# AliyunContainerService/gpushare-device-plugin

Measured on AMD Instinct MI355X. Metric: pods/sec scheduled (gpu-mem share Allocate pipeline), higher is better.
Workload: dtype n/a; 1 GPU; model=gpushare-device-plugin (MI355X), global_batch=4, seq_len=71, parallelism=1 plugin + 1 churn ranks, pods_allocated=2776, pods_failed=0

## Files before the change

__graft_entry__.py:

```python

from __future__ import annotations

import os
import sys

sys.path.insert(0, os.path.dirname(os.path.abspath(__file__)))


def build() -> None:
    os.environ.setdefault("PYTORCH_ROCM_ARCH", "gfx950")
    from gpushare_amd.native.build import build as native_build

    native_build()
    import gpushare_amd
    import gpushare_amd._amdsmi
    import gpushare_amd._devlist
    import gpushare_amd._httprt

    import gpushare_amd._canary

    print("[graft] build OK: _amdsmi, _devlist, _httprt, _canary importable")


def smoke() -> None:
    import tempfile

    import torch

    assert torch.cuda.is_available(), "torch sees no GPU"

    import gpushare_amd._canary as canary
    from gpushare_amd import consts
    from gpushare_amd.allocator import Allocator
    from gpushare_amd.cluster.kubeclient import FakeKubeClient
    from gpushare_amd.cluster.podmanager import PodManager
    from gpushare_amd.device.amdsmi_source import AmdSmiSource
    from gpushare_amd.deviceplugin.server import GPUSharePlugin
    from gpushare_amd.deviceplugin.stubkubelet import StubKubelet

    src = AmdSmiSource()
    gpus = src.devices()
    assert gpus, "no AMD GPUs enumerated"
    g0 = gpus[0]
    print(
        f"[graft] {len(gpus)} GPU(s); GPU0 uuid={g0.uuid} "
        f"vram={g0.memory_bytes >> 30} GiB render={g0.render_path}"
    )

    result = canary.probe(0, vram_probe_mb=64, bandwidth=False)
    print(f"[graft] canary: {result}")
    assert result["ok"], f"canary probe failed: {result}"

    with tempfile.TemporaryDirectory(prefix="gpushare-smoke-") as sockdir:
        kube = FakeKubeClient(node_name="smoke-node")
# ... 37 lines not shown
```

gpushare_amd/deviceplugin/server.py:

```python

from __future__ import annotations

import logging
import os
import threading
import time
from concurrent import futures
from typing import Optional

import grpc

from .. import consts, metrics
from ..device import PhysicalGPU
from ..device.fakedev import FakeDeviceTable, make_codec
from . import v1beta1 as api

log = logging.getLogger(__name__)


class GPUSharePlugin:
    def __init__(
        self,
        gpus: list[PhysicalGPU],
        allocator,
        unit: str = consts.GIB,
        resource_name: str = consts.RESOURCE_NAME,
        socket_dir: str = consts.DEVICE_PLUGIN_PATH,
        socket_name: str = consts.SERVER_SOCK_NAME,
        max_workers: int = 64,
        allow_oversize_inventory: bool = False,
        numa_topology: bool = False,
    ):
        self.gpus = gpus
        self.allocator = allocator
        self.unit = unit
        self.resource_name = resource_name
        self.socket_dir = socket_dir
        self.socket_name = socket_name
        self.socket_path = os.path.join(socket_dir, socket_name)
        self.max_workers = max_workers

        self.table = FakeDeviceTable.build(gpus, unit)
        self._codec = make_codec(
            self.table.ids,
            numa=self.table.numa_of if numa_topology else None,
        )
        metrics.observe_inventory(len(self.table))
        self.inventory_bytes = len(self._codec.encode([]))
        if self.inventory_bytes > consts.KUBELET_GRPC_MAX_MSG:
            msg = (
                f"inventory of {len(self.table)} fake devices encodes to "
                f"{self.inventory_bytes / 1e6:.1f} MB — over the kubelet's "
                f"4 MiB gRPC receive limit; use GiB granularity on "
                f"288 GiB-class GPUs (or a kubelet built with a larger "
                f"limit + allow_oversize_inventory)"
            )
            if not allow_oversize_inventory:
                raise ValueError(msg)
            log.warning("%s — continuing as requested", msg)

        self._health_lock = threading.Condition()
        self._unhealthy_gpus: set[int] = set()
        self._health_version = 0

        self._server: Optional[grpc.Server] = None
        self._stop_event = threading.Event()

    def set_gpu_health(self, gpu_index: Optional[int], healthy: bool) -> None:
        with self._health_lock:
            targets = (
                [g.index for g in self.gpus] if gpu_index is None else [gpu_index]
            )
            changed = False
            for idx in targets:
                if healthy and idx in self._unhealthy_gpus:
                    self._unhealthy_gpus.discard(idx)
                    changed = True
                elif not healthy and idx not in self._unhealthy_gpus:
                    self._unhealthy_gpus.add(idx)
                    changed = True
            if changed:
                self._health_version += 1
                self._health_lock.notify_all()
                metrics.observe_health_event(
                    "recovered" if healthy else "unhealthy",
                    len(self._unhealthy_gpus),
                )

    def _unhealthy_fake_indices(self) -> list[int]:
        out: list[int] = []
        for gpu_idx in self._unhealthy_gpus:
            out.extend(self.table.gpu_fake_indices(gpu_idx))
        return out

    def encoded_device_list(self) -> bytes:
        return self._codec.encode(self._unhealthy_fake_indices())

    def _get_options(self, request, context) -> "api.DevicePluginOptions":
# ... 44 lines not shown
                out.deviceIDs.extend(chosen[: cr.allocation_size])
                continue
            chosen_set = set(chosen)
            by_gpu: dict[int, list[str]] = {}
            for dev_id in cr.available_deviceIDs:
                if dev_id in chosen_set:
                    continue
                gpu_idx = self.table.gpu_of.get(dev_id)
                if gpu_idx is not None:
                    by_gpu.setdefault(gpu_idx, []).append(dev_id)
            fitting = sorted(
                (ids for ids in by_gpu.values() if len(ids) >= need),
                key=len,
            )
            if need and fitting:
                chosen.extend(fitting[0][:need])
            else:
                for ids in sorted(by_gpu.values(), key=len, reverse=True):
                    if need <= 0:
                        break
                    take = ids[:need]
                    chosen.extend(take)
                    need -= len(take)
            out.deviceIDs.extend(chosen)
        return resp

    def _pre_start(self, request, context) -> "api.PreStartContainerResponse":
        return api.PreStartContainerResponse()

    def start(self) -> None:
        if os.path.exists(self.socket_path):
            os.unlink(self.socket_path)
        os.makedirs(self.socket_dir, exist_ok=True)

        handlers = {
            "GetDevicePluginOptions": grpc.unary_unary_rpc_method_handler(
                self._get_options,
                request_deserializer=api.Empty.FromString,
                response_serializer=lambda m: m.SerializeToString(),
            ),
            "ListAndWatch": grpc.unary_stream_rpc_method_handler(
                self._list_and_watch,
                request_deserializer=api.Empty.FromString,
                response_serializer=None,
            ),
            "Allocate": grpc.unary_unary_rpc_method_handler(
                self._allocate,
                request_deserializer=api.AllocateRequest.FromString,
                response_serializer=lambda m: m.SerializeToString(),
            ),
            "PreStartContainer": grpc.unary_unary_rpc_method_handler(
                self._pre_start,
                request_deserializer=api.PreStartContainerRequest.FromString,
                response_serializer=lambda m: m.SerializeToString(),
            ),
            "GetPreferredAllocation": grpc.unary_unary_rpc_method_handler(
                self._get_preferred_allocation,
                request_deserializer=(
                    api.PreferredAllocationRequest.FromString
                ),
                response_serializer=lambda m: m.SerializeToString(),
            ),
        }
        self._server = grpc.server(
            futures.ThreadPoolExecutor(max_workers=self.max_workers)
        )
        self._server.add_generic_rpc_handlers(
            (
                grpc.method_handlers_generic_handler(
                    api.DEVICEPLUGIN_SERVICE, handlers
                ),
            )
        )
        self._server.add_insecure_port(f"unix://{self.socket_path}")
        self._stop_event.clear()
        self._server.start()

        with grpc.insecure_channel(f"unix://{self.socket_path}") as ch:
            grpc.channel_ready_future(ch).result(timeout=5)
        log.info("device plugin serving on %s", self.socket_path)

    def register(self, kubelet_socket: Optional[str] = None) -> None:
        if kubelet_socket is None:
            kubelet_socket = os.path.join(
                self.socket_dir, consts.KUBELET_SOCKET_NAME
            )
        req = api.RegisterRequest(
            version=consts.API_VERSION,
            endpoint=self.socket_name,
            resource_name=self.resource_name,
        )
        with grpc.insecure_channel(f"unix://{kubelet_socket}") as ch:
            grpc.channel_ready_future(ch).result(timeout=10)
            register = ch.unary_unary(
                api.METHOD_REGISTER,
                request_serializer=lambda m: m.SerializeToString(),
                response_deserializer=api.Empty.FromString,
            )
            register(req, timeout=10)
        log.info(
            "registered resource %s (%d fake devices) with kubelet at %s",
            self.resource_name,
            len(self.table),
            kubelet_socket,
        )

    def serve(self, kubelet_socket: Optional[str] = None) -> None:
        self.start()
        self.register(kubelet_socket)

    def stop(self) -> None:
        self._stop_event.set()
        with self._health_lock:
            self._health_lock.notify_all()
        if self._server is not None:
            self._server.stop(grace=1).wait(timeout=5)
            self._server = None
        if os.path.exists(self.socket_path):
            try:
                os.unlink(self.socket_path)
            except OSError:
                pass
        if hasattr(self.allocator, "close"):
            self.allocator.close()

    def wait_stopped(self, timeout: float = 5.0) -> None:
        deadline = time.monotonic() + timeout
        while self._server is not None and time.monotonic() < deadline:
            time.sleep(0.01)
```

gpushare_amd/native/build.py:

```python

from __future__ import annotations

import os
import subprocess
import sys
import sysconfig
from pathlib import Path

import pybind11

HERE = Path(__file__).resolve().parent
PKG = HERE.parent
EXT_SUFFIX = sysconfig.get_config_var("EXT_SUFFIX") or ".so"
ROCM = os.environ.get("ROCM_PATH", "/opt/rocm")
GPU_ARCH = os.environ.get("PYTORCH_ROCM_ARCH", "gfx950").split(";")[0]

_COMMON = [
    "-O2",
    "-std=c++17",
    "-fPIC",
    "-shared",
    "-fvisibility=hidden",
    f"-I{pybind11.get_include()}",
    f"-I{sysconfig.get_paths()['include']}",
]


def _needs_build(srcs: list[Path], out: Path, force: bool) -> bool:
    if force or not out.exists():
        return True
    return any(s.stat().st_mtime > out.stat().st_mtime for s in srcs)


def _run(cmd: list[str]) -> None:
    print("[native/build]", " ".join(cmd), flush=True)
    subprocess.run(cmd, check=True)


def build(force: bool = False, verbose: bool = True) -> list[Path]:
    built = []

    targets = [
        (
            "g++",
            HERE / "amdsmi_shim.cpp",
            PKG / f"_amdsmi{EXT_SUFFIX}",
            [f"-I{ROCM}/include", "-ldl"],
        ),
        ("g++", HERE / "devlist_codec.cpp", PKG / f"_devlist{EXT_SUFFIX}", []),
        ("g++", HERE / "http_rt.cpp", PKG / f"_httprt{EXT_SUFFIX}", []),
        (
            os.path.join(ROCM, "bin", "hipcc"),
            HERE / "canary.hip",
            PKG / f"_canary{EXT_SUFFIX}",
            [f"--offload-arch={GPU_ARCH}", "-O3"],
        ),
        (
            "g++",
            HERE / "memguard.cpp",
            PKG / "libgpushare_memguard.so",
            ["-fvisibility=default", "-ldl"],
        ),
    ]
    deps = {"http_rt.cpp": [HERE / "http_parse.h"]}
    for compiler, src, out, extra in targets:
        if not _needs_build([src, *deps.get(src.name, [])], out, force):
            continue
        _run([compiler, *_COMMON, str(src), "-o", str(out), *extra])
        built.append(out)
    return built


def main() -> None:
    force = "--force" in sys.argv
    built = build(force=force)
    print(f"[native/build] built {len(built)} extension(s)")
    sys.path.insert(0, str(PKG.parent))
    import gpushare_amd._amdsmi as smi
    import gpushare_amd._devlist as dl
    import gpushare_amd._httprt as rt

    print("[native/build] _amdsmi available:", smi.available())
    c = dl.DeviceListCodec(["amd-0-_-0"])
    assert len(c.encode()) > 0
    print("[native/build] _devlist OK")
    head = rt.build_head("GET", "/", "localhost", {"Accept": "*/*"})
    assert head.startswith(b"GET / HTTP/1.1\r\nHost: localhost\r\n")
    print("[native/build] _httprt OK")


if __name__ == "__main__":
    main()
```

Baseline: 2446 pods/s.

## Serve device-plugin gRPC through a native C++ HTTP/2 core instead of grpcio

Adds a pybind11 C++ extension that implements a minimal HTTP/2 + HPACK gRPC server over the Unix socket, with per-connection threads that call into Python handlers only for dispatch. The plugin uses it by default and falls back to grpcio if the module is missing or the env switch disables it. The aim is to cut grpcio's per-RPC Python and threadpool overhead on the Allocate path. In exchange it carries a hand-written protocol implementation with risks around correctness, flow control, thread lifetime and GIL handling.

```diff
diff --git a/__graft_entry__.py b/__graft_entry__.py
--- a/__graft_entry__.py
+++ b/__graft_entry__.py
@@ -15,11 +15,12 @@
     import gpushare_amd
     import gpushare_amd._amdsmi
     import gpushare_amd._devlist
+    import gpushare_amd._grpcsrv
     import gpushare_amd._httprt
 
     import gpushare_amd._canary
 
-    print("[graft] build OK: _amdsmi, _devlist, _httprt, _canary importable")
+    print("[graft] build OK: _amdsmi, _devlist, _httprt, _grpcsrv, _canary importable")
 
 
 def smoke() -> None:
diff --git a/gpushare_amd/deviceplugin/server.py b/gpushare_amd/deviceplugin/server.py
--- a/gpushare_amd/deviceplugin/server.py
+++ b/gpushare_amd/deviceplugin/server.py
@@ -16,6 +16,39 @@
 from . import v1beta1 as api
 
 log = logging.getLogger(__name__)
+
+
+def _native_core():
+    if os.environ.get("GPUSHARE_GRPC_NATIVE", "1") == "0":
+        return None
+    try:
+        from .. import _grpcsrv
+    except ImportError:
+        return None
+    return _grpcsrv
+
+
+class RpcAbort(Exception):
+
+    def __init__(self, code: int, details: str):
+        super().__init__(details)
+        self.grpc_code = code
+        self.grpc_details = details
+
+
+class _NativeContext:
+
+    __slots__ = ("_call",)
+
+    def __init__(self, call):
+        self._call = call
+
+    def is_active(self) -> bool:
+        return self._call.is_active()
+
+    def abort(self, code, details: str):
+        value = getattr(code, "value", code)
+        raise RpcAbort(value[0] if isinstance(value, tuple) else int(value), details)
 
 
 class GPUSharePlugin:
@@ -64,6 +97,7 @@
         self._health_version = 0
 
         self._server: Optional[grpc.Server] = None
+        self._native = None
         self._stop_event = threading.Event()
 
     def set_gpu_health(self, gpu_index: Optional[int], healthy: bool) -> None:
@@ -174,7 +208,62 @@
         if os.path.exists(self.socket_path):
             os.unlink(self.socket_path)
         os.makedirs(self.socket_dir, exist_ok=True)
-
+        self._stop_event.clear()
+        core = _native_core()
+        if core is not None:
+            self._start_native(core)
+        else:
+            self._start_grpcio()
+
+        with grpc.insecure_channel(f"unix://{self.socket_path}") as ch:
+            grpc.channel_ready_future(ch).result(timeout=5)
+        log.info(
+            "device plugin serving on %s (%s transport)",
+            self.socket_path,
+            "native" if self._native is not None else "grpcio",
+        )
+
+    def _start_native(self, core) -> None:
+        self._native_methods = {
+            api.METHOD_GET_OPTIONS: (
+                self._get_options, api.Empty.FromString, False),
+            api.METHOD_LIST_AND_WATCH: (
+                self._list_and_watch, api.Empty.FromString, True),
+            api.METHOD_ALLOCATE: (
+                self._allocate, api.AllocateRequest.FromString, False),
+            api.METHOD_PRE_START: (
+                self._pre_start,
+                api.PreStartContainerRequest.FromString, False),
+            api.METHOD_GET_PREFERRED: (
+                self._get_preferred_allocation,
+                api.PreferredAllocationRequest.FromString, False),
+        }
+        self._native = core.Server(
+            self.socket_path, self._native_dispatch,
+            consts.KUBELET_GRPC_MAX_MSG,
+        )
+        self._native.start()
+
+    def _native_dispatch(self, path: str, data: bytes, call):
+        method = self._native_methods.get(path)
+        if method is None:
+            raise RpcAbort(12, "Method not found!")
+        behavior, parse, streaming = method
+        try:
+            request = parse(data)
+        except Exception:
+            log.exception("Exception deserializing request!")
+            raise RpcAbort(13, "Exception deserializing request!") from None
+        try:
+            response = behavior(request, _NativeContext(call))
+        except RpcAbort:
+            raise
+        except Exception:
+            log.exception("Exception calling application")
+            raise
+        return response if streaming else response.SerializeToString()
+
+    def _start_grpcio(self) -> None:
         handlers = {
             "GetDevicePluginOptions": grpc.unary_unary_rpc_method_handler(
                 self._get_options,
@@ -215,12 +304,7 @@
             )
         )
         self._server.add_insecure_port(f"unix://{self.socket_path}")
-        self._stop_event.clear()
         self._server.start()
-
-        with grpc.insecure_channel(f"unix://{self.socket_path}") as ch:
-            grpc.channel_ready_future(ch).result(timeout=5)
-        log.info("device plugin serving on %s", self.socket_path)
 
     def register(self, kubelet_socket: Optional[str] = None) -> None:
         if kubelet_socket is None:
@@ -258,6 +342,10 @@
         if self._server is not None:
             self._server.stop(grace=1).wait(timeout=5)
             self._server = None
+        if self._native is not None:
+            if not self._native.stop(1.0):
+                log.warning("native gRPC core: threads still winding down")
+            self._native = None
         if os.path.exists(self.socket_path):
             try:
                 os.unlink(self.socket_path)
@@ -268,5 +356,7 @@
 
     def wait_stopped(self, timeout: float = 5.0) -> None:
         deadline = time.monotonic() + timeout
-        while self._server is not None and time.monotonic() < deadline:
+        while (
+            self._server is not None or self._native is not None
+        ) and time.monotonic() < deadline:
             time.sleep(0.01)
diff --git a/gpushare_amd/native/build.py b/gpushare_amd/native/build.py
--- a/gpushare_amd/native/build.py
+++ b/gpushare_amd/native/build.py
@@ -50,6 +50,12 @@
         ("g++", HERE / "devlist_codec.cpp", PKG / f"_devlist{EXT_SUFFIX}", []),
         ("g++", HERE / "http_rt.cpp", PKG / f"_httprt{EXT_SUFFIX}", []),
         (
+            "g++",
+            HERE / "grpc_srv.cpp",
+            PKG / f"_grpcsrv{EXT_SUFFIX}",
+            ["-pthread"],
+        ),
+        (
             os.path.join(ROCM, "bin", "hipcc"),
             HERE / "canary.hip",
             PKG / f"_canary{EXT_SUFFIX}",
@@ -62,7 +68,10 @@
             ["-fvisibility=default", "-ldl"],
         ),
     ]
-    deps = {"http_rt.cpp": [HERE / "http_parse.h"]}
+    deps = {
+        "http_rt.cpp": [HERE / "http_parse.h"],
+        "grpc_srv.cpp": [HERE / "h2_core.h"],
+    }
     for compiler, src, out, extra in targets:
         if not _needs_build([src, *deps.get(src.name, [])], out, force):
             continue
@@ -78,6 +87,7 @@
     sys.path.insert(0, str(PKG.parent))
     import gpushare_amd._amdsmi as smi
     import gpushare_amd._devlist as dl
+    import gpushare_amd._grpcsrv as gs
     import gpushare_amd._httprt as rt
 
     print("[native/build] _amdsmi available:", smi.available())
@@ -87,6 +97,9 @@
     head = rt.build_head("GET", "/", "localhost", {"Accept": "*/*"})
     assert head.startswith(b"GET / HTTP/1.1\r\nHost: localhost\r\n")
     print("[native/build] _httprt OK")
+    block = bytes.fromhex("828684418cf1e3c2e5f23a6ba0ab90f4ff")
+    assert gs.hpack_decode(block)[3] == (b":authority", b"www.example.com")
+    print("[native/build] _grpcsrv OK")
 
 
 if __name__ == "__main__":
diff --git a/gpushare_amd/native/grpc_srv.cpp b/gpushare_amd/native/grpc_srv.cpp
--- /dev/null
+++ b/gpushare_amd/native/grpc_srv.cpp
@@ -0,0 +1,524 @@
+
+#include <pybind11/pybind11.h>
+
+#include <poll.h>
+#include <sys/socket.h>
+#include <sys/time.h>
+#include <sys/types.h>
+#include <sys/un.h>
+#include <unistd.h>
+#include <fcntl.h>
+
+#include <algorithm>
+#include <cerrno>
+#include <chrono>
+#include <condition_variable>
+#include <cstring>
+#include <memory>
+#include <mutex>
+#include <string>
+#include <thread>
+#include <vector>
+
+#include "h2_core.h"
+
+namespace py = pybind11;
+
+namespace {
+
+constexpr size_t kMaxConnections = 64;
+constexpr size_t kRecvBuf = 64 * 1024;
+constexpr size_t kStreamBacklog = 256 * 1024;
+constexpr int kSendTimeoutS = 5;
+
+inline bool finalizing() {
+#if PY_VERSION_HEX >= 0x030D0000
+  return Py_IsFinalizing() != 0;
+#else
+  return _Py_IsFinalizing() != 0;
+#endif
+}
+
+class PyThread {
+ public:
+  PyThread() {
+    park_if_finalizing();
+    gs_ = PyGILState_Ensure();
+    ts_ = PyEval_SaveThread();
+  }
+  ~PyThread() {
+    acquire();
+    PyGILState_Release(gs_);
+  }
+  PyThread(const PyThread &) = delete;
+  PyThread &operator=(const PyThread &) = delete;
+
+  void acquire() {
+    park_if_finalizing();
+    PyEval_RestoreThread(ts_);
+  }
+  void release() { ts_ = PyEval_SaveThread(); }
+
+ private:
+  static void park_if_finalizing() {
+    if (finalizing())
+      for (;;) pause();
+  }
+  PyGILState_STATE gs_;
+  PyThreadState *ts_;
+};
+
+struct Conn {
+  Conn(int fd_, size_t max_message) : fd(fd_), core(max_message) {}
+  const int fd;
+  std::mutex mu;
+  std::mutex wmu;
+  std::condition_variable cv;
+  h2::Connection core;
+  std::string wbuf;
+  bool closing = false;
+  int stream_threads = 0;
+};
+
+struct Shared {
+  std::mutex mu;
+  std::condition_variable cv;
+  std::vector<std::shared_ptr<Conn>> conns;
+  int threads = 0;
+  bool stopping = false;
+  PyObject *handler = nullptr;
+  size_t max_message = 0;
+};
+
+void thread_done(const std::shared_ptr<Shared> &sh) {
+  {
+    std::lock_guard<std::mutex> g(sh->mu);
+    --sh->threads;
+  }
+  sh->cv.notify_all();
+}
+
+void flush(Conn &c) {
+  std::lock_guard<std::mutex> w(c.wmu);
+  c.wbuf.clear();
+  {
+    std::lock_guard<std::mutex> g(c.mu);
+    c.wbuf.swap(c.core.out());
+  }
+  size_t off = 0;
+  while (off < c.wbuf.size()) {
+    ssize_t n = ::send(c.fd, c.wbuf.data() + off, c.wbuf.size() - off,
+                       MSG_NOSIGNAL);
+    if (n > 0) {
+      off += static_cast<size_t>(n);
+      continue;
+    }
+    if (n < 0 && errno == EINTR) continue;
+    {
+      std::lock_guard<std::mutex> g(c.mu);
+      c.closing = true;
+    }
+    ::shutdown(c.fd, SHUT_RDWR);
+    c.cv.notify_all();
+    return;
+  }
+}
+
+struct Call {
+  std::shared_ptr<Conn> conn;
+  uint32_t stream;
+  bool is_active() const {
+    std::lock_guard<std::mutex> g(conn->mu);
+    return !conn->closing && conn->core.alive(stream);
+  }
+};
+
+void status_of(py::error_already_set &e, int &status, std::string &text) {
+  status = h2::kUnknown;
+  try {
+    py::object v = e.value();
+    if (!v.is_none() && py::hasattr(v, "grpc_code")) {
+      status = v.attr("grpc_code").cast<int>();
+      text = py::str(v.attr("grpc_details")).cast<std::string>();
+      return;
+    }
+    text = "Exception calling application: " +
+           py::str(v).cast<std::string>();
+  } catch (py::error_already_set &inner) {
+    inner.discard_as_unraisable("gpushare_amd._grpcsrv");
+    status = h2::kUnknown;
+    text = "Exception calling application";
+  }
+}
+
+void finish_and_flush(Conn &c, uint32_t id, int status,
+                      const std::string &text) {
+  {
+    std::lock_guard<std::mutex> g(c.mu);
+    c.core.finish(id, status, text);
+  }
+  flush(c);
+}
+
+void run_stream(std::shared_ptr<Shared> sh, std::shared_ptr<Conn> c,
+                uint32_t id, PyObject *iter) {
+  {
+    PyThread pt;
+    int status = h2::kOk;
+    std::string text, data;
+    bool cancelled = false;
+    for (;;) {
+      bool done = false;
+      pt.acquire();
+      PyObject *item = PyIter_Next(iter);
+      if (item == nullptr) {
+        done = true;
+        if (PyErr_Occurred()) {
+          py::error_already_set e;
+          status_of(e, status, text);
+        }
+      } else if (PyBytes_Check(item)) {
+        data.assign(PyBytes_AS_STRING(item),
+                    static_cast<size_t>(PyBytes_GET_SIZE(item)));
+      } else {
+        done = true;
+        status = h2::kInternal;
+        text = "Failed to serialize response!";
+      }
+      Py_XDECREF(item);
+      pt.release();
+      if (done) break;
+      {
+        std::lock_guard<std::mutex> g(c->mu);
+        if (c->closing || !c->core.alive(id))
+          cancelled = true;
+        else
+          c->core.send_message(id, data.data(), data.size());
+      }
+      if (cancelled) break;
+      flush(*c);
+      std::unique_lock<std::mutex> lk(c->mu);
+      c->cv.wait(lk, [&] {
+        return c->closing || !c->core.alive(id) ||
+               c->core.pending(id) <= kStreamBacklog;
+      });
+    }
+    pt.acquire();
+    if (cancelled) {
+      PyObject *r = PyObject_CallMethod(iter, "close", nullptr);
+      if (r == nullptr) PyErr_Clear();
+      Py_XDECREF(r);
+    }
+    Py_DECREF(iter);
+    pt.release();
+    if (!cancelled) finish_and_flush(*c, id, status, text);
+    {
+      std::lock_guard<std::mutex> g(c->mu);
+      --c->stream_threads;
+    }
+    c->cv.notify_all();
+  }
+  thread_done(sh);
+}
+
+void handle_request(const std::shared_ptr<Shared> &sh,
+                    const std::shared_ptr<Conn> &c,
+                    std::unique_ptr<PyThread> &pt, h2::Event &ev) {
+  if (!pt) pt.reset(new PyThread());
+  int status = h2::kOk;
+  std::string text, data;
+  PyObject *iter = nullptr;
+  pt->acquire();
+  try {
+    py::object result = py::reinterpret_borrow<py::object>(sh->handler)(
+        py::str(ev.path), py::bytes(ev.message), Call{c, ev.stream});
+    if (PyBytes_Check(result.ptr())) {
+      data.assign(PyBytes_AS_STRING(result.ptr()),
+                  static_cast<size_t>(PyBytes_GET_SIZE(result.ptr())));
+    } else {
+      iter = PyObject_GetIter(result.ptr());
+      if (iter == nullptr) throw py::error_already_set();
+    }
+  } catch (py::error_already_set &e) {
+    status_of(e, status, text);
+  }
+  pt->release();
+
+  if (iter != nullptr) {
+    bool started = false;
+    {
+      std::lock_guard<std::mutex> g(sh->mu);
+      std::lock_guard<std::mutex> g2(c->mu);
+      try {
+        ++sh->threads;
+        ++c->stream_threads;
+        std::thread(run_stream, sh, c, ev.stream, iter).detach();
+        started = true;
+      } catch (const std::system_error &) {
+        --sh->threads;
+        --c->stream_threads;
+      }
+    }
+    if (started) return;
+    pt->acquire();
+    Py_DECREF(iter);
+    pt->release();
+    status = h2::kResourceExhausted;
+    text = "cannot start a thread for the stream";
+  }
+  {
+    std::lock_guard<std::mutex> g(c->mu);
+    if (status == h2::kOk) c->core.send_message(ev.stream, data.data(), data.size());
+    c->core.finish(ev.stream, status, text);
+  }
+  flush(*c);
+}
+
+void serve_conn(std::shared_ptr<Shared> sh, std::shared_ptr<Conn> c) {
+  {
+    std::unique_ptr<PyThread> pt;
+    {
+      std::lock_guard<std::mutex> g(c->mu);
+      c->core.start();
+    }
+    flush(*c);
+    std::vector<uint8_t> buf(kRecvBuf);
+    std::vector<h2::Event> events;
+    for (;;) {
+      ssize_t n = ::recv(c->fd, buf.data(), buf.size(), 0);
+      if (n < 0 && errno == EINTR) continue;
+      if (n <= 0) break;
+      bool ok;
+      events.clear();
+      {
+        std::lock_guard<std::mutex> g(c->mu);
+        ok = c->core.feed(buf.data(), static_cast<size_t>(n));
+        events.swap(c->core.events());
+      }
+      flush(*c);
+      c->cv.notify_all();
+      for (h2::Event &ev : events)
+        if (ev.type == h2::Event::request) handle_request(sh, c, pt, ev);
+      if (!ok) break;
+      std::lock_guard<std::mutex> g(c->mu);
+      if (c->closing) break;
+    }
+    {
+      std::lock_guard<std::mutex> g(c->mu);
+      c->closing = true;
+      c->core.goaway(h2::kNoError);
+    }
+    c->cv.notify_all();
+    flush(*c);
+    ::shutdown(c->fd, SHUT_RDWR);
+    {
+      std::unique_lock<std::mutex> lk(c->mu);
+      c->cv.wait(lk, [&] { return c->stream_threads == 0; });
+    }
+    {
+      std::lock_guard<std::mutex> g(sh->mu);
+      ::close(c->fd);
+      sh->conns.erase(std::remove(sh->conns.begin(), sh->conns.end(), c),
+                      sh->conns.end());
+    }
+  }
+  thread_done(sh);
+}
+
+void accept_loop(std::shared_ptr<Shared> sh, int lfd, int wake_r) {
+  for (;;) {
+    struct pollfd p[2] = {{lfd, POLLIN, 0}, {wake_r, POLLIN, 0}};
+    int r = ::poll(p, 2, -1);
+    if (r < 0 && errno == EINTR) continue;
+    if (r < 0 || p[1].revents != 0) break;
+    int fd = ::accept4(lfd, nullptr, nullptr, SOCK_CLOEXEC);
+    if (fd < 0) {
+      if (errno == EINTR || errno == EAGAIN || errno == ECONNABORTED) continue;
+      if (errno == EMFILE || errno == ENFILE || errno == ENOMEM) {
+        ::poll(nullptr, 0, 50);
+        continue;
+      }
+      break;
+    }
+    struct timeval tv = {kSendTimeoutS, 0};
+    ::setsockopt(fd, SOL_SOCKET, SO_SNDTIMEO, &tv, sizeof tv);
+    std::lock_guard<std::mutex> g(sh->mu);
+    if (sh->stopping || sh->conns.size() >= kMaxConnections) {
+      ::close(fd);
+      continue;
+    }
+    try {
+      auto c = std::make_shared<Conn>(fd, sh->max_message);
+      sh->conns.push_back(c);
+      ++sh->threads;
+      try {
+        std::thread(serve_conn, sh, c).detach();
+      } catch (const std::system_error &) {
+        --sh->threads;
+        sh->conns.pop_back();
+        ::close(fd);
+      }
+    } catch (const std::bad_alloc &) {
+      ::close(fd);
+    }
+  }
+  ::close(lfd);
+  ::close(wake_r);
+  thread_done(sh);
+}
+
+class Server {
+ public:
+  Server(std::string path, py::object handler, size_t max_message)
+      : path_(std::move(path)), sh_(std::make_shared<Shared>()) {
+    if (path_.size() >= sizeof(sockaddr_un{}.sun_path))
+      throw py::value_error("unix socket path too long");
+    sh_->handler = handler.release().ptr();
+    sh_->max_message = max_message;
+  }
+
+  ~Server() {
+    if (started_ && !stopped_) stop(0.0);
+    release_handler();
+  }
+
+  void start() {
+    if (started_) throw std::runtime_error("server already started");
+    int lfd = ::socket(AF_UNIX, SOCK_STREAM | SOCK_CLOEXEC, 0);
+    if (lfd < 0) raise_errno();
+    struct sockaddr_un addr;
+    std::memset(&addr, 0, sizeof addr);
+    addr.sun_family = AF_UNIX;
+    std::memcpy(addr.sun_path, path_.data(), path_.size());
+    int pipefd[2] = {-1, -1};
+    if (::bind(lfd, reinterpret_cast<struct sockaddr *>(&addr), sizeof addr) <
+            0 ||
+        ::listen(lfd, 128) < 0 || ::pipe2(pipefd, O_CLOEXEC) < 0) {
+      int e = errno;
+      ::close(lfd);
+      errno = e;
+      raise_errno();
+    }
+    wake_w_ = pipefd[1];
+    {
+      std::lock_guard<std::mutex> g(sh_->mu);
+      ++sh_->threads;
+    }
+    try {
+      std::thread(accept_loop, sh_, lfd, pipefd[0]).detach();
+    } catch (const std::system_error &) {
+      {
+        std::lock_guard<std::mutex> g(sh_->mu);
+        --sh_->threads;
+      }
+      ::close(lfd);
+      ::close(pipefd[0]);
+      ::close(wake_w_);
+      wake_w_ = -1;
+      throw;
+    }
+    started_ = true;
+  }
+
+  bool stop(double grace) {
+    if (!started_ || stopped_) return true;
+    stopped_ = true;
+    {
+      std::lock_guard<std::mutex> g(sh_->mu);
+      sh_->stopping = true;
+      for (auto &c : sh_->conns) {
+        {
+          std::lock_guard<std::mutex> g2(c->mu);
+          c->core.goaway(h2::kNoError);
+          c->closing = true;
+        }
+        c->cv.notify_all();
+        ::shutdown(c->fd, SHUT_RD);
+      }
+    }
+    char b = 1;
+    while (::write(wake_w_, &b, 1) < 0 && errno == EINTR) {
+    }
+    ::close(wake_w_);
+    wake_w_ = -1;
+    bool all_gone;
+    {
+      py::gil_scoped_release nogil;
+      std::unique_lock<std::mutex> lk(sh_->mu);
+      all_gone = sh_->cv.wait_for(
+          lk, std::chrono::duration<double>(grace < 0 ? 0.0 : grace),
+          [&] { return sh_->threads == 0; });
+    }
+    if (all_gone) release_handler();
+    return all_gone;
+  }
+
+  size_t connections() const {
+    std::lock_guard<std::mutex> g(sh_->mu);
+    return sh_->conns.size();
+  }
+
+  int threads() const {
+    std::lock_guard<std::mutex> g(sh_->mu);
+    return sh_->threads;
+  }
+
+ private:
+  [[noreturn]] static void raise_errno() {
+    PyErr_SetFromErrno(PyExc_OSError);
+    throw py::error_already_set();
+  }
+
+  void release_handler() {
+    std::lock_guard<std::mutex> g(sh_->mu);
+    if (sh_->threads == 0 && sh_->handler != nullptr) {
+      Py_DECREF(sh_->handler);
+      sh_->handler = nullptr;
+    }
+  }
+
+  std::string path_;
+  std::shared_ptr<Shared> sh_;
+  int wake_w_ = -1;
+  bool started_ = false, stopped_ = false;
+};
+
+py::list hpack_decode(py::bytes block) {
+  char *p;
+  Py_ssize_t n;
+  if (PyBytes_AsStringAndSize(block.ptr(), &p, &n) < 0)
+    throw py::error_already_set();
+  h2::HpackDecoder dec;
+  std::vector<h2::Header> headers;
+  h2::HpackError e = dec.decode(reinterpret_cast<const uint8_t *>(p),
+                                static_cast<size_t>(n), headers, 1u << 20);
+  if (e != h2::HpackError::none)
+    throw py::value_error("HPACK error " + std::to_string(static_cast<int>(e)));
+  py::list out;
+  for (const h2::Header &h : headers)
+    out.append(py::make_tuple(py::bytes(h.name), py::bytes(h.value)));
+  return out;
+}
+
+}
+
+PYBIND11_MODULE(_grpcsrv, m) {
+  m.doc() = "gRPC-over-HTTP/2 server core for the device-plugin socket";
+
+  py::class_<Call>(m, "Call")
+      .def("is_active", &Call::is_active)
+      .def_readonly("stream", &Call::stream);
+
+  py::class_<Server>(m, "Server")
+      .def(py::init<std::string, py::object, size_t>(), py::arg("path"),
+           py::arg("handler"), py::arg("max_message") = size_t(4) << 20)
+      .def("start", &Server::start)
+      .def("stop", &Server::stop, py::arg("grace") = 1.0)
+      .def_property_readonly("connections", &Server::connections)
+      .def_property_readonly("threads", &Server::threads);
+
+  m.def("hpack_decode", &hpack_decode, py::arg("block"));
+  m.attr("MAX_CONCURRENT_STREAMS") = h2::kMaxConcurrentStreams;
+  m.attr("MAX_CONNECTIONS") = kMaxConnections;
+  m.attr("MAX_HEADER_LIST") = h2::kMaxHeaderList;
+}
diff --git a/gpushare_amd/native/h2_core.h b/gpushare_amd/native/h2_core.h
--- /dev/null
+++ b/gpushare_amd/native/h2_core.h
@@ -0,0 +1,1001 @@
+
+#pragma once
+
+#include <cstddef>
+#include <cstdint>
+#include <cstring>
+#include <deque>
+#include <map>
+#include <string>
+#include <utility>
+#include <vector>
+
+namespace h2 {
+
+enum FrameType : uint8_t {
+  kData = 0, kHeaders = 1, kPriority = 2, kRstStream = 3, kSettings = 4,
+  kPushPromise = 5, kPing = 6, kGoaway = 7, kWindowUpdate = 8,
+  kContinuation = 9,
+};
+enum Flag : uint8_t {
+  kEndStream = 0x1, kAck = 0x1, kEndHeaders = 0x4, kPadded = 0x8,
+  kPriorityFlag = 0x20,
+};
+enum ErrorCode : uint32_t {
+  kNoError = 0, kProtocolError = 1, kInternalError = 2, kFlowControlError = 3,
+  kSettingsTimeout = 4, kStreamClosed = 5, kFrameSizeError = 6,
+  kRefusedStream = 7, kCancel = 8, kCompressionError = 9,
+  kEnhanceYourCalm = 0xb,
+};
+enum GrpcStatus : int {
+  kOk = 0, kUnknown = 2, kResourceExhausted = 8, kUnimplemented = 12,
+  kInternal = 13,
+};
+
+constexpr size_t kFrameHeaderLen = 9;
+constexpr size_t kPrefaceLen = 24;
+constexpr char kPreface[] = "PRI * HTTP/2.0\r\n\r\nSM\r\n\r\n";
+constexpr int64_t kDefaultWindow = 65535;
+constexpr int64_t kMaxWindow = 0x7fffffff;
+constexpr uint32_t kDefaultMaxFrame = 16384;
+constexpr uint32_t kMaxMaxFrame = 16777215;
+
+constexpr uint32_t kOurMaxFrame = 16384;
+constexpr uint32_t kOurHeaderTable = 4096;
+constexpr uint32_t kMaxConcurrentStreams = 128;
+constexpr uint32_t kMaxHeaderList = 16 * 1024;
+constexpr int64_t kOurStreamWindow = 1 << 20;
+constexpr int64_t kOurConnWindow = 4 << 20;
+constexpr size_t kMaxGrpcMessageText = 1024;
+
+constexpr uint8_t kHuffBits[257] = {
+    13, 23, 28, 28, 28, 28, 28, 28, 28, 24, 30, 28, 28, 30, 28, 28,
+    28, 28, 28, 28, 28, 28, 30, 28, 28, 28, 28, 28, 28, 28, 28, 28,
+     6, 10, 10, 12, 13,  6,  8, 11, 10, 10,  8, 11,  8,  6,  6,  6,
+     5,  5,  5,  6,  6,  6,  6,  6,  6,  6,  7,  8, 15,  6, 12, 10,
+    13,  6,  7,  7,  7,  7,  7,  7,  7,  7,  7,  7,  7,  7,  7,  7,
+     7,  7,  7,  7,  7,  7,  7,  7,  8,  7,  8, 13, 19, 13, 14,  6,
+    15,  5,  6,  5,  6,  5,  6,  6,  6,  5,  7,  7,  6,  6,  6,  5,
+     6,  7,  6,  5,  5,  6,  7,  7,  7,  7,  7, 15, 11, 14, 13, 28,
+    20, 22, 20, 20, 22, 22, 22, 23, 22, 23, 23, 23, 23, 23, 24, 23,
+    24, 24, 22, 23, 24, 23, 23, 23, 23, 21, 22, 23, 22, 23, 23, 24,
+    22, 21, 20, 22, 22, 23, 23, 21, 23, 22, 22, 24, 21, 22, 23, 23,
+    21, 21, 22, 21, 23, 22, 23, 23, 20, 22, 22, 22, 23, 22, 22, 23,
+    26, 26, 20, 19, 22, 23, 22, 25, 26, 26, 26, 27, 27, 26, 24, 25,
+    19, 21, 26, 27, 27, 26, 27, 24, 21, 21, 26, 26, 28, 27, 27, 27,
+    20, 24, 20, 21, 22, 21, 21, 23, 22, 22, 25, 25, 24, 24, 26, 23,
+    26, 27, 26, 26, 27, 27, 27, 27, 27, 28, 27, 27, 27, 27, 27, 26,
+    30,
+};
+constexpr int kHuffEos = 256;
+
+class Huffman {
+ public:
+  static const Huffman &get() {
+    static const Huffman h;
+    return h;
+  }
+
+  uint32_t code(int sym) const { return code_[sym]; }
+  int bits(int sym) const { return kHuffBits[sym]; }
+
+  bool decode(const uint8_t *p, size_t n, std::string &out) const {
+    int node = 0, depth = 0;
+    bool ones = true;
+    for (size_t i = 0; i < n; ++i) {
+      for (int b = 7; b >= 0; --b) {
+        int bit = (p[i] >> b) & 1;
+        node = next_[node][bit];
+        ++depth;
+        ones = ones && bit;
+        if (node < 0) {
+          int sym = -node - 1;
+          if (sym == kHuffEos) return false;
+          out.push_back(static_cast<char>(sym));
+          node = 0;
+          depth = 0;
+          ones = true;
+        }
+      }
+    }
+    return depth <= 7 && ones;
+  }
+
+  void encode(const uint8_t *p, size_t n, std::string &out) const {
+    uint64_t acc = 0;
+    int have = 0;
+    for (size_t i = 0; i < n; ++i) {
+      acc = (acc << kHuffBits[p[i]]) | code_[p[i]];
+      have += kHuffBits[p[i]];
+      while (have >= 8) {
+        out.push_back(static_cast<char>((acc >> (have - 8)) & 0xff));
+        have -= 8;
+      }
+    }
+    if (have > 0) {
+      uint64_t pad = (1u << (8 - have)) - 1;
+      out.push_back(static_cast<char>(((acc << (8 - have)) | pad) & 0xff));
+    }
+  }
+
+ private:
+  Huffman() {
+    uint32_t next_code = 0;
+    for (int len = 5; len <= 30; ++len) {
+      for (int s = 0; s <= kHuffEos; ++s)
+        if (kHuffBits[s] == len) code_[s] = next_code++;
+      next_code <<= 1;
+    }
+    std::memset(next_, 0, sizeof next_);
+    int nodes = 1;
+    for (int s = 0; s <= kHuffEos; ++s) {
+      int node = 0;
+      for (int b = kHuffBits[s] - 1; b >= 0; --b) {
+        int bit = (code_[s] >> b) & 1;
+        if (b == 0) {
+          next_[node][bit] = static_cast<int16_t>(-(s + 1));
+        } else {
+          if (next_[node][bit] == 0)
+            next_[node][bit] = static_cast<int16_t>(nodes++);
+          node = next_[node][bit];
+        }
+      }
+    }
+  }
+
+  uint32_t code_[257];
+  int16_t next_[256][2];
+};
+
+struct Header {
+  std::string name, value;
+};
+
+struct StaticEntry {
+  const char *name, *value;
+};
+constexpr StaticEntry kStaticTable[61] = {
+    {":authority", ""}, {":method", "GET"}, {":method", "POST"},
+    {":path", "/"}, {":path", "/index.html"}, {":scheme", "http"},
+    {":scheme", "https"}, {":status", "200"}, {":status", "204"},
+    {":status", "206"}, {":status", "304"}, {":status", "400"},
+    {":status", "404"}, {":status", "500"}, {"accept-charset", ""},
+    {"accept-encoding", "gzip, deflate"}, {"accept-language", ""},
+    {"accept-ranges", ""}, {"accept", ""},
+    {"access-control-allow-origin", ""}, {"age", ""}, {"allow", ""},
+    {"authorization", ""}, {"cache-control", ""},
+    {"content-disposition", ""}, {"content-encoding", ""},
+    {"content-language", ""}, {"content-length", ""},
+    {"content-location", ""}, {"content-range", ""}, {"content-type", ""},
+    {"cookie", ""}, {"date", ""}, {"etag", ""}, {"expect", ""},
+    {"expires", ""}, {"from", ""}, {"host", ""}, {"if-match", ""},
+    {"if-modified-since", ""}, {"if-none-match", ""}, {"if-range", ""},
+    {"if-unmodified-since", ""}, {"last-modified", ""}, {"link", ""},
+    {"location", ""}, {"max-forwards", ""}, {"proxy-authenticate", ""},
+    {"proxy-authorization", ""}, {"range", ""}, {"referer", ""},
+    {"refresh", ""}, {"retry-after", ""}, {"server", ""},
+    {"set-cookie", ""}, {"strict-transport-security", ""},
+    {"transfer-encoding", ""}, {"user-agent", ""}, {"vary", ""}, {"via", ""},
+    {"www-authenticate", ""},
+};
+constexpr uint32_t kStaticCount = 61;
+constexpr int kStaticStatus = 8;
+constexpr int kStaticContentType = 31;
+
+enum class HpackError {
+  none,
+  truncated,
+  bad_integer,
+  bad_index,
+  bad_huffman,
+  bad_size_update,
+  too_large,
+};
+
+inline bool hpack_decode_int(const uint8_t *&p, const uint8_t *end, int prefix,
+                             uint32_t &v, HpackError &err) {
+  if (p == end) {
+    err = HpackError::truncated;
+    return false;
+  }
+  const uint32_t mask = (1u << prefix) - 1;
+  v = *p++ & mask;
+  if (v < mask) return true;
+  for (int shift = 0;; shift += 7) {
+    if (p == end) {
+      err = HpackError::truncated;
+      return false;
+    }
+    if (shift > 21) {
+      err = HpackError::bad_integer;
+      return false;
+    }
+    uint8_t b = *p++;
+    v += static_cast<uint32_t>(b & 0x7f) << shift;
+    if (!(b & 0x80)) return true;
+  }
+}
+
+inline void hpack_encode_int(std::string &out, uint8_t first, int prefix,
+                             uint32_t v) {
+  const uint32_t mask = (1u << prefix) - 1;
+  if (v < mask) {
+    out.push_back(static_cast<char>(first | v));
+    return;
+  }
+  out.push_back(static_cast<char>(first | mask));
+  v -= mask;
+  while (v >= 128) {
+    out.push_back(static_cast<char>((v & 0x7f) | 0x80));
+    v >>= 7;
+  }
+  out.push_back(static_cast<char>(v));
+}
+
+inline void hpack_encode_literal(std::string &out, int name_index,
+                                 const char *name, const std::string &value) {
+  hpack_encode_int(out, 0x00, 4, static_cast<uint32_t>(name_index));
+  if (name_index == 0) {
+    size_t n = std::strlen(name);
+    hpack_encode_int(out, 0x00, 7, static_cast<uint32_t>(n));
+    out.append(name, n);
+  }
+  hpack_encode_int(out, 0x00, 7, static_cast<uint32_t>(value.size()));
+  out.append(value);
+}
+
+class HpackDecoder {
+ public:
+  explicit HpackDecoder(uint32_t cap = kOurHeaderTable)
+      : cap_(cap), max_size_(cap) {}
+
+  HpackError decode(const uint8_t *p, size_t n, std::vector<Header> &out,
+                    size_t max_list) {
+    const uint8_t *end = p + n;
+    HpackError err = HpackError::none;
+    bool seen_field = false;
+    size_t list_size = 0;
+    while (p < end) {
+      uint8_t b = *p;
+      Header h;
+      if (b & 0x80) {
+        uint32_t idx;
+        if (!hpack_decode_int(p, end, 7, idx, err)) return err;
+        if (!lookup(idx, h, true)) return HpackError::bad_index;
+      } else if ((b & 0xe0) == 0x20) {
+        uint32_t size;
+        if (!hpack_decode_int(p, end, 5, size, err)) return err;
+        if (seen_field || size > cap_) return HpackError::bad_size_update;
+        max_size_ = size;
+        evict(0);
+        continue;
+      } else {
+        const bool index_it = (b & 0xc0) == 0x40;
+        uint32_t idx;
+        if (!hpack_decode_int(p, end, index_it ? 6 : 4, idx, err)) return err;
+        if (idx != 0) {
+          if (!lookup(idx, h, false)) return HpackError::bad_index;
+        } else if (!decode_string(p, end, h.name, err)) {
+          return err;
+        }
+        if (!decode_string(p, end, h.value, err)) return err;
+        if (index_it) insert(h);
+      }
+      seen_field = true;
+      list_size += h.name.size() + h.value.size() + 32;
+      if (list_size > max_list) return HpackError::too_large;
+      out.push_back(std::move(h));
+    }
+    return HpackError::none;
+  }
+
+  size_t dyn_count() const { return dyn_.size(); }
+  size_t dyn_size() const { return dyn_size_; }
+  const Header &dyn_entry(size_t i) const { return dyn_[i]; }
+  uint32_t max_size() const { return max_size_; }
+
+ private:
+  bool lookup(uint32_t idx, Header &h, bool with_value) const {
+    if (idx == 0) return false;
+    if (idx <= kStaticCount) {
+      h.name = kStaticTable[idx - 1].name;
+      if (with_value) h.value = kStaticTable[idx - 1].value;
+      return true;
+    }
+    size_t d = idx - kStaticCount - 1;
+    if (d >= dyn_.size()) return false;
+    h.name = dyn_[d].name;
+    if (with_value) h.value = dyn_[d].value;
+    return true;
+  }
+
+  static bool decode_string(const uint8_t *&p, const uint8_t *end,
+                            std::string &out, HpackError &err) {
+    if (p == end) {
+      err = HpackError::truncated;
+      return false;
+    }
+    const bool huff = (*p & 0x80) != 0;
+    uint32_t len;
+    if (!hpack_decode_int(p, end, 7, len, err)) return false;
+    if (len > static_cast<size_t>(end - p)) {
+      err = HpackError::truncated;
+      return false;
+    }
+    if (huff) {
+      if (!Huffman::get().decode(p, len, out)) {
+        err = HpackError::bad_huffman;
+        return false;
+      }
+    } else {
+      out.assign(reinterpret_cast<const char *>(p), len);
+    }
+    p += len;
+    return true;
+  }
+
+  void evict(size_t incoming) {
+    while (!dyn_.empty() && dyn_size_ + incoming > max_size_) {
+      dyn_size_ -= dyn_.back().name.size() + dyn_.back().value.size() + 32;
+      dyn_.pop_back();
+    }
+  }
+
+  void insert(const Header &h) {
+    size_t sz = h.name.size() + h.value.size() + 32;
+    evict(sz);
+    if (sz > max_size_) return;
+    dyn_.push_front(h);
+    dyn_size_ += sz;
+  }
+
+  uint32_t cap_;
+  uint32_t max_size_;
+  size_t dyn_size_ = 0;
+  std::deque<Header> dyn_;
+};
+
+inline void put_u32(std::string &out, uint32_t v) {
+  char b[4] = {static_cast<char>(v >> 24), static_cast<char>(v >> 16),
+               static_cast<char>(v >> 8), static_cast<char>(v)};
+  out.append(b, 4);
+}
+
+inline uint32_t get_u32(const uint8_t *p) {
+  return (static_cast<uint32_t>(p[0]) << 24) |
+         (static_cast<uint32_t>(p[1]) << 16) |
+         (static_cast<uint32_t>(p[2]) << 8) | p[3];
+}
+
+inline void put_frame_header(std::string &out, size_t len, uint8_t type,
+                             uint8_t flags, uint32_t stream) {
+  char b[9] = {static_cast<char>(len >> 16), static_cast<char>(len >> 8),
+               static_cast<char>(len), static_cast<char>(type),
+               static_cast<char>(flags), static_cast<char>((stream >> 24) & 0x7f),
+               static_cast<char>(stream >> 16), static_cast<char>(stream >> 8),
+               static_cast<char>(stream)};
+  out.append(b, 9);
+}
+
+inline std::string percent_encode(const std::string &s) {
+  static const char hex[] = "0123456789ABCDEF";
+  std::string out;
+  for (unsigned char c : s) {
+    if (c >= 0x20 && c <= 0x7e && c != '%') {
+      out.push_back(static_cast<char>(c));
+    } else {
+      out.push_back('%');
+      out.push_back(hex[c >> 4]);
+      out.push_back(hex[c & 15]);
+    }
+  }
+  return out;
+}
+
+inline int64_t parse_grpc_timeout(const std::string &s) {
+  if (s.size() < 2 || s.size() > 9) return -1;
+  int64_t v = 0;
+  for (size_t i = 0; i + 1 < s.size(); ++i) {
+    if (s[i] < '0' || s[i] > '9') return -1;
+    v = v * 10 + (s[i] - '0');
+  }
+  int64_t unit;
+  switch (s.back()) {
+    case 'H': unit = 3600 * 1000000000LL; break;
+    case 'M': unit = 60 * 1000000000LL; break;
+    case 'S': unit = 1000000000LL; break;
+    case 'm': unit = 1000000LL; break;
+    case 'u': unit = 1000LL; break;
+    case 'n': unit = 1; break;
+    default: return -1;
+  }
+  if (v > INT64_MAX / unit) return INT64_MAX;
+  return v * unit;
+}
+
+struct Event {
+  enum Type { request, reset } type;
+  uint32_t stream;
+  std::string path;
+  std::string message;
+  int64_t timeout_ns;
+};
+
+class Connection {
+ public:
+  explicit Connection(size_t max_message) : max_message_(max_message) {}
+
+  void start() {
+    put_frame_header(out_, 18, kSettings, 0, 0);
+    put_setting(3, kMaxConcurrentStreams);
+    put_setting(4, static_cast<uint32_t>(kOurStreamWindow));
+    put_setting(6, kMaxHeaderList);
+    put_frame_header(out_, 4, kWindowUpdate, 0, 0);
+    put_u32(out_, static_cast<uint32_t>(kOurConnWindow - kDefaultWindow));
+    conn_recv_window_ = kOurConnWindow;
+  }
+
+  bool feed(const uint8_t *p, size_t n) {
+    if (failed_) return false;
+    in_.append(reinterpret_cast<const char *>(p), n);
+    size_t off = 0;
+    while (!failed_) {
+      const uint8_t *d = reinterpret_cast<const uint8_t *>(in_.data()) + off;
+      size_t avail = in_.size() - off;
+      if (!preface_done_) {
+        size_t k = avail < kPrefaceLen ? avail : kPrefaceLen;
+        if (std::memcmp(d, kPreface, k) != 0) {
+          conn_error(kProtocolError);
+          break;
+        }
+        if (avail < kPrefaceLen) break;
+        preface_done_ = true;
+        off += kPrefaceLen;
+        continue;
+      }
+      if (avail < kFrameHeaderLen) break;
+      uint32_t len = (static_cast<uint32_t>(d[0]) << 16) |
+                     (static_cast<uint32_t>(d[1]) << 8) | d[2];
+      if (len > kOurMaxFrame) {
+        conn_error(kFrameSizeError);
+        break;
+      }
+      if (avail < kFrameHeaderLen + len) break;
+      on_frame(d[3], d[4], get_u32(d + 5) & 0x7fffffff, d + kFrameHeaderLen,
+               len);
+      off += kFrameHeaderLen + len;
+    }
+    in_.erase(0, off);
+    return !failed_;
+  }
+
+  std::vector<Event> &events() { return events_; }
+  std::string &out() { return out_; }
+  bool failed() const { return failed_; }
+  uint32_t error() const { return error_; }
+  bool goaway_received() const { return goaway_received_; }
+
+  bool alive(uint32_t id) const { return !failed_ && streams_.count(id) != 0; }
+
+  size_t pending(uint32_t id) const {
+    auto it = streams_.find(id);
+    if (it == streams_.end()) return 0;
+    return it->second.pending.size() - it->second.pending_off;
+  }
+
+  void send_message(uint32_t id, const char *data, size_t n) {
+    auto it = streams_.find(id);
+    if (it == streams_.end() || failed_) return;
+    Stream &s = it->second;
+    if (s.finishing) return;
+    send_response_headers(id, s);
+    compact(s);
+    char prefix[5] = {0, static_cast<char>(n >> 24), static_cast<char>(n >> 16),
+                      static_cast<char>(n >> 8), static_cast<char>(n)};
+    s.pending.append(prefix, 5);
+    s.pending.append(data, n);
+    pump(id);
+  }
+
+  void finish(uint32_t id, int status, const std::string &message) {
+    auto it = streams_.find(id);
+    if (it == streams_.end() || failed_) return;
+    Stream &s = it->second;
+    if (s.finishing) return;
+    s.finishing = true;
+    s.trailers.clear();
+    if (!s.headers_sent) {
+      begin_block(s.trailers);
+      hpack_encode_literal(s.trailers, kStaticStatus, "", "200");
+      hpack_encode_literal(s.trailers, kStaticContentType, "",
+                           "application/grpc");
+      s.headers_sent = true;
+    }
+    hpack_encode_literal(s.trailers, 0, "grpc-status", std::to_string(status));
+    if (!message.empty()) {
+      std::string m = message.size() > kMaxGrpcMessageText
+                          ? message.substr(0, kMaxGrpcMessageText)
+                          : message;
+      hpack_encode_literal(s.trailers, 0, "grpc-message", percent_encode(m));
+    }
+    pump(id);
+  }
+
+  void goaway(uint32_t code) {
+    if (goaway_sent_) return;
+    goaway_sent_ = true;
+    put_frame_header(out_, 8, kGoaway, 0, 0);
+    put_u32(out_, last_stream_);
+    put_u32(out_, code);
+  }
+
+  int64_t conn_send_window() const { return conn_send_window_; }
+  int64_t conn_recv_window() const { return conn_recv_window_; }
+  uint32_t peer_max_frame() const { return peer_max_frame_; }
+  size_t stream_count() const { return streams_.size(); }
+  const HpackDecoder &hpack() const { return hpack_; }
+
+ private:
+  struct Stream {
+    int64_t send_window = 0;
+    int64_t recv_window = kOurStreamWindow;
+    int64_t recv_unacked = 0;
+    bool remote_closed = false;
+    bool headers_sent = false;
+    bool finishing = false;
+    std::string path;
+    int64_t timeout_ns = -1;
+    std::string body;
+    std::string pending;
+    size_t pending_off = 0;
+    std::string trailers;
+  };
+
+  void put_setting(uint16_t id, uint32_t v) {
+    out_.push_back(static_cast<char>(id >> 8));
+    out_.push_back(static_cast<char>(id));
+    put_u32(out_, v);
+  }
+
+  bool conn_error(uint32_t code) {
+    goaway(code);
+    failed_ = true;
+    error_ = code;
+    streams_.clear();
+    return false;
+  }
+
+  void rst_stream(uint32_t id, uint32_t code) {
+    put_frame_header(out_, 4, kRstStream, 0, id);
+    put_u32(out_, code);
+  }
+
+  void stream_error(uint32_t id, uint32_t code) {
+    rst_stream(id, code);
+    if (streams_.erase(id)) events_.push_back(Event{Event::reset, id, "", "", -1});
+  }
+
+  void begin_block(std::string &block) {
+    if (table_update_due_) {
+      block.push_back(0x20);
+      table_update_due_ = false;
+    }
+  }
+
+  void send_response_headers(uint32_t id, Stream &s) {
+    if (s.headers_sent) return;
+    s.headers_sent = true;
+    std::string block;
+    begin_block(block);
+    hpack_encode_literal(block, kStaticStatus, "", "200");
+    hpack_encode_literal(block, kStaticContentType, "", "application/grpc");
+    put_frame_header(out_, block.size(), kHeaders, kEndHeaders, id);
+    out_.append(block);
+  }
+
+  static void compact(Stream &s) {
+    if (s.pending_off == s.pending.size()) {
+      s.pending.clear();
+      s.pending_off = 0;
+    }
+  }
+
+  void pump(uint32_t id) {
+    auto it = streams_.find(id);
+    if (it == streams_.end()) return;
+    Stream &s = it->second;
+    while (s.pending_off < s.pending.size()) {
+      int64_t n = static_cast<int64_t>(s.pending.size() - s.pending_off);
+      if (n > peer_max_frame_) n = peer_max_frame_;
+      if (n > conn_send_window_) n = conn_send_window_;
+      if (n > s.send_window) n = s.send_window;
+      if (n <= 0) return;
+      put_frame_header(out_, static_cast<size_t>(n), kData, 0, id);
+      out_.append(s.pending, s.pending_off, static_cast<size_t>(n));
+      s.pending_off += static_cast<size_t>(n);
+      conn_send_window_ -= n;
+      s.send_window -= n;
+    }
+    if (!s.finishing) return;
+    put_frame_header(out_, s.trailers.size(), kHeaders,
+                     kEndHeaders | kEndStream, id);
+    out_.append(s.trailers);
+    if (!s.remote_closed) rst_stream(id, kNoError);
+    streams_.erase(it);
+  }
+
+  void pump_all() {
+    std::vector<uint32_t> ids;
+    for (auto &kv : streams_)
+      if (kv.second.pending_off < kv.second.pending.size()) ids.push_back(kv.first);
+    for (uint32_t id : ids) pump(id);
+  }
+
+  void reject(uint32_t id, int status, const std::string &message) {
+    auto it = streams_.find(id);
+    if (it == streams_.end()) return;
+    it->second.pending.clear();
+    it->second.pending_off = 0;
+    finish(id, status, message);
+  }
+
+  void on_frame(uint8_t type, uint8_t flags, uint32_t id, const uint8_t *p,
+                uint32_t len) {
+    if (!settings_seen_ && type != kSettings) {
+      conn_error(kProtocolError);
+      return;
+    }
+    if (continuation_of_ != 0 &&
+        (type != kContinuation || id != continuation_of_)) {
+      conn_error(kProtocolError);
+      return;
+    }
+    switch (type) {
+      case kData: on_data(flags, id, p, len); break;
+      case kHeaders: on_headers(flags, id, p, len); break;
+      case kContinuation: on_continuation(flags, id, p, len); break;
+      case kPriority:
+        if (id == 0) conn_error(kProtocolError);
+        else if (len != 5) stream_error(id, kFrameSizeError);
+        break;
+      case kRstStream: on_rst_stream(id, len); break;
+      case kSettings: on_settings(flags, id, p, len); break;
+      case kPushPromise: conn_error(kProtocolError); break;
+      case kPing:
+        if (id != 0) {
+          conn_error(kProtocolError);
+        } else if (len != 8) {
+          conn_error(kFrameSizeError);
+        } else if (!(flags & kAck)) {
+          put_frame_header(out_, 8, kPing, kAck, 0);
+          out_.append(reinterpret_cast<const char *>(p), 8);
+        }
+        break;
+      case kGoaway:
+        if (id != 0) conn_error(kProtocolError);
+        else if (len < 8) conn_error(kFrameSizeError);
+        else goaway_received_ = true;
+        break;
+      case kWindowUpdate: on_window_update(id, p, len); break;
+      default: break;
+    }
+  }
+
+  void on_settings(uint8_t flags, uint32_t id, const uint8_t *p, uint32_t len) {
+    if (id != 0) {
+      conn_error(kProtocolError);
+      return;
+    }
+    if (flags & kAck) {
+      if (len != 0) conn_error(kFrameSizeError);
+      return;
+    }
+    if (len % 6 != 0) {
+      conn_error(kFrameSizeError);
+      return;
+    }
+    for (uint32_t i = 0; i < len; i += 6) {
+      uint16_t key = static_cast<uint16_t>((p[i] << 8) | p[i + 1]);
+      uint32_t v = get_u32(p + i + 2);
+      switch (key) {
+        case 1:
+          table_update_due_ = true;
+          break;
+        case 2:
+          if (v > 1) {
+            conn_error(kProtocolError);
+            return;
+          }
+          break;
+        case 4: {
+          if (v > kMaxWindow) {
+            conn_error(kFlowControlError);
+            return;
+          }
+          int64_t delta = static_cast<int64_t>(v) - peer_initial_window_;
+          peer_initial_window_ = v;
+          for (auto &kv : streams_) {
+            kv.second.send_window += delta;
+            if (kv.second.send_window > kMaxWindow) {
+              conn_error(kFlowControlError);
+              return;
+            }
+          }
+          break;
+        }
+        case 5:
+          if (v < kDefaultMaxFrame || v > kMaxMaxFrame) {
+            conn_error(kProtocolError);
+            return;
+          }
+          peer_max_frame_ = v;
+          break;
+        default: break;
+      }
+    }
+    settings_seen_ = true;
+    put_frame_header(out_, 0, kSettings, kAck, 0);
+    pump_all();
+  }
+
+  void on_window_update(uint32_t id, const uint8_t *p, uint32_t len) {
+    if (len != 4) {
+      conn_error(kFrameSizeError);
+      return;
+    }
+    int64_t inc = get_u32(p) & 0x7fffffff;
+    if (id == 0) {
+      if (inc == 0) {
+        conn_error(kProtocolError);
+      } else if (conn_send_window_ + inc > kMaxWindow) {
+        conn_error(kFlowControlError);
+      } else {
+        conn_send_window_ += inc;
+        pump_all();
+      }
+      return;
+    }
+    if (is_idle(id)) {
+      conn_error(kProtocolError);
+      return;
+    }
+    auto it = streams_.find(id);
+    if (it == streams_.end()) return;
+    if (inc == 0) {
+      stream_error(id, kProtocolError);
+    } else if (it->second.send_window + inc > kMaxWindow) {
+      stream_error(id, kFlowControlError);
+    } else {
+      it->second.send_window += inc;
+      pump(id);
+    }
+  }
+
+  void on_rst_stream(uint32_t id, uint32_t len) {
+    if (len != 4) {
+      conn_error(kFrameSizeError);
+      return;
+    }
+    if (id == 0 || is_idle(id)) {
+      conn_error(kProtocolError);
+      return;
+    }
+    if (streams_.erase(id)) events_.push_back(Event{Event::reset, id, "", "", -1});
+  }
+
+  bool is_idle(uint32_t id) const { return (id & 1) == 0 || id > highest_stream_; }
+
+  bool strip(uint8_t flags, bool priority_allowed, const uint8_t *&p,
+             uint32_t &len) {
+    uint32_t pad = 0;
+    if (flags & kPadded) {
+      if (len < 1) return conn_error(kFrameSizeError);
+      pad = p[0];
+      ++p;
+      --len;
+    }
+    if (priority_allowed && (flags & kPriorityFlag)) {
+      if (len < 5) return conn_error(kFrameSizeError);
+      p += 5;
+      len -= 5;
+    }
+    if (pad > len) return conn_error(kProtocolError);
+    len -= pad;
+    return true;
+  }
+
+  void on_data(uint8_t flags, uint32_t id, const uint8_t *p, uint32_t len) {
+    if (id == 0 || is_idle(id)) {
+      conn_error(kProtocolError);
+      return;
+    }
+    const uint32_t flow = len;
+    if (!strip(flags, false, p, len)) return;
+    conn_recv_window_ -= flow;
+    if (conn_recv_window_ < 0) {
+      conn_error(kFlowControlError);
+      return;
+    }
+    conn_recv_unacked_ += flow;
+    if (conn_recv_unacked_ >= kOurConnWindow / 2) {
+      put_frame_header(out_, 4, kWindowUpdate, 0, 0);
+      put_u32(out_, static_cast<uint32_t>(conn_recv_unacked_));
+      conn_recv_window_ += conn_recv_unacked_;
+      conn_recv_unacked_ = 0;
+    }
+    auto it = streams_.find(id);
+    if (it == streams_.end()) return;
+    Stream &s = it->second;
+    if (s.remote_closed) {
+      stream_error(id, kStreamClosed);
+      return;
+    }
+    s.recv_window -= flow;
+    if (s.recv_window < 0) {
+      stream_error(id, kFlowControlError);
+      return;
+    }
+    const bool end = (flags & kEndStream) != 0;
+    s.recv_unacked += flow;
+    if (!end && s.recv_unacked >= kOurStreamWindow / 2) {
+      put_frame_header(out_, 4, kWindowUpdate, 0, id);
+      put_u32(out_, static_cast<uint32_t>(s.recv_unacked));
+      s.recv_window += s.recv_unacked;
+      s.recv_unacked = 0;
+    }
+    if (s.finishing) return;
+    const size_t before = s.body.size();
+    s.body.append(reinterpret_cast<const char *>(p), len);
+    if (before < 5 && s.body.size() >= 5) {
+      const uint8_t *b = reinterpret_cast<const uint8_t *>(s.body.data());
+      if (b[0] != 0) {
+        reject(id, kUnimplemented, "compressed request messages are not supported");
+        return;
+      }
+      if (get_u32(b + 1) > max_message_) {
+        reject(id, kResourceExhausted,
+               "Received message larger than max (" +
+                   std::to_string(get_u32(b + 1)) + " vs. " +
+                   std::to_string(max_message_) + ")");
+        return;
+      }
+    }
+    if (s.body.size() >= 5) {
+      const uint8_t *b = reinterpret_cast<const uint8_t *>(s.body.data());
+      if (s.body.size() > 5 + static_cast<size_t>(get_u32(b + 1))) {
+        reject(id, kUnimplemented, "client-streaming calls are not supported");
+        return;
+      }
+    }
+    if (end) on_remote_end(id, s);
+  }
+
+  void on_remote_end(uint32_t id, Stream &s) {
+    s.remote_closed = true;
+    if (s.body.size() < 5 ||
+        s.body.size() !=
+            5 + static_cast<size_t>(get_u32(
+                    reinterpret_cast<const uint8_t *>(s.body.data()) + 1))) {
+      reject(id, kInternal, "request message missing or truncated");
+      return;
+    }
+    Event ev{Event::request, id, s.path, s.body.substr(5), s.timeout_ns};
+    std::string().swap(s.body);
+    events_.push_back(std::move(ev));
+  }
+
+  void on_headers(uint8_t flags, uint32_t id, const uint8_t *p, uint32_t len) {
+    if (id == 0) {
+      conn_error(kProtocolError);
+      return;
+    }
+    if (!strip(flags, true, p, len)) return;
+    block_.assign(reinterpret_cast<const char *>(p), len);
+    block_end_stream_ = (flags & kEndStream) != 0;
+    if (flags & kEndHeaders) {
+      on_block_complete(id);
+    } else {
+      continuation_of_ = id;
+    }
+  }
+
+  void on_continuation(uint8_t flags, uint32_t id, const uint8_t *p,
+                       uint32_t len) {
+    if (continuation_of_ == 0 || id != continuation_of_) {
+      conn_error(kProtocolError);
+      return;
+    }
+    block_.append(reinterpret_cast<const char *>(p), len);
+    if (block_.size() > kMaxHeaderList) {
+      conn_error(kEnhanceYourCalm);
+      return;
+    }
+    if (flags & kEndHeaders) {
+      continuation_of_ = 0;
+      on_block_complete(id);
+    }
+  }
+
+  void on_block_complete(uint32_t id) {
+    std::vector<Header> headers;
+    HpackError e =
+        hpack_.decode(reinterpret_cast<const uint8_t *>(block_.data()),
+                      block_.size(), headers, kMaxHeaderList);
+    block_.clear();
+    if (e != HpackError::none) {
+      conn_error(e == HpackError::too_large ? kEnhanceYourCalm
+                                            : kCompressionError);
+      return;
+    }
+    auto it = streams_.find(id);
+    if (it != streams_.end()) {
+      if (!block_end_stream_ || it->second.remote_closed) {
+        stream_error(id, kProtocolError);
+        return;
+      }
+      on_remote_end(id, it->second);
+      return;
+    }
+    if ((id & 1) == 0) {
+      conn_error(kProtocolError);
+      return;
+    }
+    if (id <= highest_stream_) {
+      return;
+    }
+    highest_stream_ = id;
+    if (goaway_sent_) return;
+    last_stream_ = id;
+    if (streams_.size() >= kMaxConcurrentStreams) {
+      rst_stream(id, kRefusedStream);
+      return;
+    }
+    Stream &s = streams_[id];
+    s.send_window = peer_initial_window_;
+    std::string method, content_type;
+    for (Header &h : headers) {
+      if (h.name == ":path") s.path = std::move(h.value);
+      else if (h.name == ":method") method = std::move(h.value);
+      else if (h.name == "content-type") content_type = std::move(h.value);
+      else if (h.name == "grpc-timeout") s.timeout_ns = parse_grpc_timeout(h.value);
+    }
+    if (method != "POST" || s.path.empty()) {
+      stream_error(id, kProtocolError);
+      return;
+    }
+    if (content_type.compare(0, 16, "application/grpc") != 0) {
+      std::string block;
+      begin_block(block);
+      hpack_encode_literal(block, kStaticStatus, "", "415");
+      put_frame_header(out_, block.size(), kHeaders, kEndHeaders | kEndStream,
+                       id);
+      out_.append(block);
+      if (!block_end_stream_) rst_stream(id, kNoError);
+      streams_.erase(id);
+      return;
+    }
+    if (block_end_stream_) on_remote_end(id, s);
+  }
+
+  const size_t max_message_;
+  std::string in_, out_;
+  std::vector<Event> events_;
+  std::map<uint32_t, Stream> streams_;
+  HpackDecoder hpack_;
+  std::string block_;
+  bool block_end_stream_ = false;
+  uint32_t continuation_of_ = 0;
+  uint32_t last_stream_ = 0;
+  uint32_t highest_stream_ = 0;
+  bool preface_done_ = false, settings_seen_ = false;
+  bool failed_ = false, goaway_sent_ = false, goaway_received_ = false;
+  bool table_update_due_ = false;
+  uint32_t error_ = kNoError;
+  int64_t conn_send_window_ = kDefaultWindow;
+  int64_t conn_recv_window_ = kDefaultWindow;
+  int64_t conn_recv_unacked_ = 0;
+  int64_t peer_initial_window_ = kDefaultWindow;
+  uint32_t peer_max_frame_ = kDefaultMaxFrame;
+};
+
+}
```

After: 2381 pods/s. 2.7% lower.
